# dog-qiuqiu/Yolo-FastestV2

Measured on AMD Instinct MI355X. Metric: images/sec at 352x352 bs=256 per GPU (forward+decode+NMS), higher is better.
Workload: dtype f32 tensors; contractions fp16x3 (two-term fp16 split operands on v_mfma_f32_16x16x32_f16, fp32 accumulate); depthwise/BN/ReLU/decode/NMS fp32 VALU; 1 GPU

## Files before the change

### yolo_fastestv2_amd/csrc/yfv2_block.hip

```cpp
#include <cstdlib>
#include <type_traits>

#include "yfv2_device.h"

template <int C2>
struct S1Cfg {
  static constexpr int KC = (C2 + 15) / 16;
  static constexpr int DW_FL = 9 * KC * 16;
  static constexpr int CST_FL = 6 * KC * 16;
};

constexpr int CH_TBL_FL = 64;

constexpr int CH6_WP_FL = 3 * 3 * 256;
constexpr int CH6_IMG_FL = 2 * CH6_WP_FL + S1Cfg<48>::DW_FL + S1Cfg<48>::CST_FL + CH_TBL_FL;

__host__ __device__ constexpr int s1chain_pitch(int PW) { return 2 * (PW + 1) + ((PW - 2 * (PW + 1)) % 16 + 16) % 16; }
__host__ __device__ constexpr int s1chain_plane(int PH, int PW) { return (2 * (PH + 1) * s1chain_pitch(PW) + 15) & ~15; }

template <int THREADS>
__global__ __launch_bounds__(THREADS, 2) void block_s1chain6_kernel(BlockS1Args a) {
  constexpr int C2 = 48;
  using Cfg = S1Cfg<C2>;
  constexpr int KC = Cfg::KC, NQ = C2 / 4, C = 2 * C2, NT = 4;
// ... 66 lines not shown
#undef CH6_EACH
  };

  auto phase_a = [&]() __attribute__((always_inline)) {
    BOps b[NT];
    int slo[NT];
#pragma unroll
    for (int n = 0; n < NT; ++n) slo[n] = opq(sl[n]);
#pragma unroll
    for (int n = 0; n < NT; ++n) {
      f32x4 bf[KC];
#pragma unroll
      for (int s2 = 0; s2 < KC; ++s2) bf[s2] = *reinterpret_cast<const f32x4*>(Tg + ((size_t)(4 * s2) * PL + slo[n]) * 4);
      b[n] = make_b(bf[0], bf[1], bf[2]);
    }
#pragma unroll
    for (int mt = 0; mt < KC; ++mt) {
      f32x4 acc[NT];
#pragma unroll
      for (int n = 0; n < NT; ++n) acc[n] = (f32x4){0.f, 0.f, 0.f, 0.f};
      mfma9(W1P, mt, b, acc);
      if (mt == 0) { watch.see(acc[0][0]); watch.see(acc[1][0]); watch.see(acc[2][0]); watch.see(acc[3][0]); }
      const f32x4 sc1 = *reinterpret_cast<const f32x4*>(CS + 0 * KC * 16 + 16 * mt + 4 * g);
      const f32x4 sh1 = *reinterpret_cast<const f32x4*>(CS + 1 * KC * 16 + 16 * mt + 4 * g);
      if (pvalid) {
#pragma unroll
        for (int n = 0; n < NT; ++n) {
          f32x4 y;
#pragma unroll
          for (int c = 0; c < 4; ++c) {
            const float uu = __builtin_fmaf(acc[n][c], sc1[c], sh1[c]);
            y[c] = uu > 0.f ? uu : 0.f;
          }
          *reinterpret_cast<f32x4*>(T1 + ((size_t)(4 * mt + g) * PL + slo[n]) * 4) = y;
        }
      }
      __builtin_amdgcn_sched_barrier(0);
    }
  };
  const int wro[4] = {0, (PH + 1) * RPT, RPT, (PH + 2) * RPT};
  const int wco[4] = {0, CP1, 1, CP1 + 1};
  auto phase_b = [&](f32x4 (&bo)[KC][NT]) __attribute__((always_inline)) {
    f32x4 dwv[KC][NT];
    const int wb = opq(wbase);
#pragma unroll
    for (int s = 0; s < KC; ++s) {
      const int cb = 16 * s + 4 * g;
      f32x4 wl[9];
#pragma unroll
      for (int k = 0; k < 9; ++k) wl[k] = *reinterpret_cast<const f32x4*>(WD + k * KC * 16 + cb);
      const f32x4 lsc = *reinterpret_cast<const f32x4*>(CS + 2 * KC * 16 + cb);
      const f32x4 lsh = *reinterpret_cast<const f32x4*>(CS + 3 * KC * 16 + cb);
      const float* pl = Tg + ((size_t)(4 * s) * PL + wb) * 4;
      f32x4 d[NT];
#pragma unroll
      for (int n = 0; n < NT; ++n) d[n] = (f32x4){0.f, 0.f, 0.f, 0.f};
#pragma unroll
      for (int wr = 0; wr < 4; ++wr) {
        f32x4 row[4];
#pragma unroll
        for (int wc = 0; wc < 4; ++wc) row[wc] = *reinterpret_cast<const f32x4*>(pl + (size_t)(wro[wr] + wco[wc]) * 4);
#pragma unroll
        for (int dy = 0; dy < 2; ++dy) {
          const int ky = wr - dy;
          if (ky < 0 || ky > 2) continue;
#pragma unroll
          for (int dx = 0; dx < 2; ++dx)
#pragma unroll
            for (int kx = 0; kx < 3; ++kx)
              d[2 * dy + dx] = __builtin_elementwise_fma(row[dx + kx], wl[3 * ky + kx], d[2 * dy + dx]);
        }
      }
#pragma unroll
      for (int n = 0; n < NT; ++n) dwv[s][n] = __builtin_elementwise_fma(d[n], lsc, lsh);
      __builtin_amdgcn_sched_barrier(0);
    }
    BOps b[NT];
#pragma unroll
    for (int n = 0; n < NT; ++n) b[n] = make_b(dwv[0][n], dwv[1][n], dwv[2][n]);
#pragma unroll
    for (int mt = 0; mt < KC; ++mt) {
      f32x4 acc[NT];
#pragma unroll
      for (int n = 0; n < NT; ++n) acc[n] = (f32x4){0.f, 0.f, 0.f, 0.f};
      mfma9(W2P, mt, b, acc);
      if (mt == 0) { watch.see(acc[0][0]); watch.see(acc[1][0]); watch.see(acc[2][0]); watch.see(acc[3][0]); }
      const f32x4 sc = *reinterpret_cast<const f32x4*>(CS + 4 * KC * 16 + 16 * mt + 4 * g);
      const f32x4 sh = *reinterpret_cast<const f32x4*>(CS + 5 * KC * 16 + 16 * mt + 4 * g);
#pragma unroll
      for (int n = 0; n < NT; ++n)
#pragma unroll
        for (int k = 0; k < 4; ++k) {
          const float u = __builtin_fmaf(acc[n][k], sc[k], sh[k]);
          bo[mt][n][k] = u > 0.f ? u : 0.f;
        }
      __builtin_amdgcn_sched_barrier(0);
    }
  };
  auto write_tile = [&](int nt, f32x4 q0, f32x4 q1, f32x4 q2) __attribute__((always_inline)) {
    if (!real[nt]) { q0 = (f32x4){0.f, 0.f, 0.f, 0.f}; q1 = q0; q2 = q0; }
    const int so = opq(sl[nt]);
    *reinterpret_cast<f32x4*>(T1 + ((size_t)(0 + g) * PL + so) * 4) = q0;
    *reinterpret_cast<f32x4*>(T1 + ((size_t)(4 + g) * PL + so) * 4) = q1;
    *reinterpret_cast<f32x4*>(T1 + ((size_t)(8 + g) * PL + so) * 4) = q2;
  };
  auto tbl = [&](int i) __attribute__((always_inline)) {
    return reinterpret_cast<const int*>(IM + 2 * CH6_WP_FL + Cfg::DW_FL + Cfg::CST_FL)[i * 4 + g];
  };
  constexpr int P1_4 = CH6_WP_FL / 4, P2_4 = (CH6_IMG_FL - CH6_WP_FL) / 4;
  constexpr int NI1 = (P1_4 + THREADS - 1) / THREADS, NI2 = (P2_4 + THREADS - 1) / THREADS;
  auto part_issue = [&](int kb_next, int off4, int n4, auto& regs) __attribute__((always_inline)) {
    const f32x4* src = reinterpret_cast<const f32x4*>(a.img + (size_t)(kb_next < NB ? kb_next : 0) * CH6_IMG_FL) + off4;
#pragma unroll
    for (int k = 0; k < (int)(sizeof(regs) / sizeof(regs[0])); ++k) { const int i = tid + k * THREADS; regs[k] = src[i < n4 ? i : n4 - 1]; }
  };
  auto part_commit = [&](int off4, int n4, const auto& regs) __attribute__((always_inline)) {
    __builtin_amdgcn_s_waitcnt(0x0F70);
#pragma unroll
    for (int k = 0; k < (int)(sizeof(regs) / sizeof(regs[0])); ++k) { const int i = tid + k * THREADS; if (i < n4) reinterpret_cast<f32x4*>(IM)[off4 + i] = regs[k]; }
  };

  for (int b = blockIdx.x; b < a.B; b += gridDim.x) {
    const float* ximg = a.in + (size_t)b * HW * C;
    float* zimg = a.out + (size_t)b * HW * C;
    float* pimg = a.park + (size_t)b * NPARK * PP4;
    float hold2[6][NT];
    {
      f32x4 xq[NT][6];
#pragma unroll
      for (int nt = 0; nt < NT; ++nt)
#pragma unroll
        for (int c = 0; c < 6; ++c)
          xq[nt][c] = *reinterpret_cast<const f32x4*>(ximg + (size_t)pix[nt] * C + 16 * c + 4 * g);
      {
        f32x4 i1[NI1], i2[NI2];
        part_issue(0, 0, P1_4, i1);
        part_issue(0, P1_4, P2_4, i2);
        __builtin_amdgcn_sched_barrier(0);
        part_commit(0, P1_4, i1);
        part_commit(P1_4, P2_4, i2);
      }
#pragma unroll
      for (int nt = 0; nt < NT; ++nt) {
        if (!real[nt]) {
#pragma unroll
          for (int c = 0; c < 6; ++c) xq[nt][c] = (f32x4){0.f, 0.f, 0.f, 0.f};
        }
        if (valid[nt]) {
#pragma unroll
          for (int j = 0; j < KC; ++j)
            *reinterpret_cast<f32x4*>(T1 + ((size_t)(4 * j + g) * PL + sl[nt]) * 4) = (f32x4){xq[nt][2 * j][1], xq[nt][2 * j][3], xq[nt][2 * j + 1][1], xq[nt][2 * j + 1][3]};
        }
#pragma unroll
        for (int c = 0; c < 6; ++c) hold2[c][nt] = xq[nt][c][2];
      }
      YFV2_WSTAMP(12);
      lds_barrier();
      YFV2_WSTAMP(13);
#pragma unroll
      for (int c = 0; c < 6; ++c) {
        const int pos = tbl(3 + c);
        if (pvalid) {
          if (pos < NPARK) {
            *reinterpret_cast<f32x4*>(pimg + (size_t)pos * PP4 + 4 * patch) = (f32x4){xq[0][c][0], xq[1][c][0], xq[2][c][0], xq[3][c][0]};
          } else {
#pragma unroll
            for (int nt = 0; nt < NT; ++nt) zimg[(size_t)pix[nt] * C + pos] = xq[nt][c][0];
          }
        }
      }
    }
    YFV2_WSTAMP(1);

    f32x4 bo[KC][NT];
    float Hd[KC][NT];
    auto run_block = [&](const int kb, auto first_tag) __attribute__((always_inline)) {
      constexpr bool FIRST = decltype(first_tag)::value;
      const bool more = kb + 1 < NB;
      {
        f32x4 n1[NI1];
        part_issue(kb + 1, 0, P1_4, n1);
        __builtin_amdgcn_sched_barrier(0);
        phase_a();
        __builtin_amdgcn_sched_barrier(0);
        if (kb == 1) YFV2_WSTAMP(6);
        if (FIRST) YFV2_WSTAMP(2);
        lds_barrier();
        if (kb == 1) YFV2_WSTAMP(7);
        if (FIRST) YFV2_WSTAMP(3);
        __builtin_amdgcn_s_waitcnt(0x0F70);
        if (more) part_commit(0, P1_4, n1);
      }
      const int ps0 = tbl(0), ps1 = tbl(1), ps2 = tbl(2);
      f32x4 n2[NI2];
      part_issue(kb + 1, P1_4, P2_4, n2);
      float plq[3][NT];
      if constexpr (!FIRST) {
        if (more) {
#pragma unroll
          for (int i = 0; i < 3; ++i) {
            const float* rec = pimg + (size_t)(12 * (kb - 1) + 3 * g + i) * PP4;
#pragma unroll
            for (int nt = 0; nt < NT; ++nt) plq[i][nt] = rec[opq(4 * patch + nt)];
          }
        }
      }
      __builtin_amdgcn_sched_barrier(0);
      phase_b(bo);
      if (kb == 1) YFV2_WSTAMP(8);
      if (FIRST) YFV2_WSTAMP(4);
      __builtin_amdgcn_s_waitcnt(0x0F70);
      if (more) {
        lds_barrier();
        part_commit(P1_4, P2_4, n2);
#pragma unroll
        for (int nt = 0; nt < NT; ++nt) {
          if (valid[nt]) {
            if constexpr (FIRST)
              write_tile(nt, (f32x4){hold2[0][nt], hold2[1][nt], hold2[2][nt], hold2[3][nt]},
                         (f32x4){hold2[4][nt], hold2[5][nt], bo[0][nt][1], bo[0][nt][3]},
                         (f32x4){bo[1][nt][1], bo[1][nt][3], bo[2][nt][1], bo[2][nt][3]});
            else
              write_tile(nt, (f32x4){Hd[0][nt], Hd[1][nt], Hd[2][nt], plq[0][nt]},
                         (f32x4){plq[1][nt], plq[2][nt], bo[0][nt][1], bo[0][nt][3]},
                         (f32x4){bo[1][nt][1], bo[1][nt][3], bo[2][nt][1], bo[2][nt][3]});
          }
#pragma unroll
          for (int mt = 0; mt < KC; ++mt) Hd[mt][nt] = bo[mt][nt][0];
        }
        if (pvalid) {
          const int ps[3] = {ps0, ps1, ps2};
#pragma unroll
          for (int i = 0; i < 3; ++i) {
            if (ps[i] < NPARK) {
              *reinterpret_cast<f32x4*>(pimg + (size_t)ps[i] * PP4 + 4 * patch) = (f32x4){bo[i][0][2], bo[i][1][2], bo[i][2][2], bo[i][3][2]};
            } else {
#pragma unroll
              for (int nt = 0; nt < NT; ++nt) zimg[(size_t)pix[nt] * C + ps[i]] = bo[i][nt][2];
            }
          }
        }
        lds_barrier();
        if (kb == 1) YFV2_WSTAMP(9);
        if (FIRST) YFV2_WSTAMP(5);
      }
    };
    run_block(0, std::true_type{});
#pragma unroll 1
    for (int kb = 1; kb < NB; ++kb) run_block(kb, std::false_type{});
    YFV2_WSTAMP(10);
#pragma unroll
    for (int nt = 0; nt < NT; ++nt)
      if (real[nt]) {
        float* zp = zimg + (size_t)pix[nt] * C;
#pragma unroll
        for (int mt = 0; mt < KC; ++mt) *reinterpret_cast<f32x4*>(zp + 16 * mt + 4 * g) = bo[mt][nt];
#pragma unroll
        for (int mt = 0; mt < KC; ++mt) zp[C2 + 3 * g + mt] = Hd[mt][nt];
      }
    YFV2_WSTAMP(11);
    __syncthreads();
  }
  watch.report(a.nonfinite);
}

static long s1chain_lds_floats(int H, int W) {
  const long pl = s1chain_plane(H / 2, W / 2);
  return (long)CH6_IMG_FL + 12L * pl * 4;
}

long yfv2_s1chain_park_floats(int H, int W, int nblk) { return 12L * (nblk - 2) * ((((H / 2) * (W / 2) + 15) & ~15) * 4); }

int yfv2_s1chain_image_floats() { return CH6_IMG_FL; }

bool yfv2_s1chain_supported(int c2, int H, int W) {
  if (c2 != 48 || H < 2 || (H & 1) || (W & 1)) return false;
  if ((H / 2) * (W / 2) > 16 * 8) return false;
  if (yfv2_s1chain_park_floats(H, W, 7) > 24L * (4 * H) * (4 * W)) return false;
  return s1chain_lds_floats(H, W) * 4 <= YFV2_LDS_FULL;
}

bool yfv2_launch_block_s1chain(const BlockS1Args& a, hipStream_t s) {
  if (!yfv2_s1chain_supported(48, a.H, a.W) || a.nblk < 2) return false;
  const size_t lds = sizeof(float) * (size_t)s1chain_lds_floats(a.H, a.W);
  const Yfv2Device dev = yfv2_device();
  YFV2_LAUNCH_LDS(dev, (block_s1chain6_kernel<512>), YFV2_LDS_FULL, dim3(yfv2_image_grid(a.B, dev)), dim3(512), lds, s, a);
  return true;
}

constexpr int P96_C2 = 96, P96_C = 192, P96_KC = 6, P96_TH = 3, P96_TC = 32;
constexpr int P96_CPP = P96_C + 4;
constexpr int P96_TP = P96_TC + 4;
constexpr int P96_W1_FL = 2 * P96_KC * 256, P96_W2_FL = P96_KC * 2 * 256;
constexpr int P96_IMG_FL = P96_W1_FL + P96_W2_FL + 9 * P96_TC + 4 * P96_TC + 2 * P96_C2;
constexpr int P96_W1P_FL = 2 * (P96_KC / 2) * 2 * 256, P96_W2P_FL = P96_KC * 1 * 2 * 256;
constexpr int P96_IMGP_FL = P96_W1P_FL + P96_W2P_FL + 9 * P96_TC + 4 * P96_TC + 2 * P96_C2;
constexpr int P96_MAXPX = 128;

template <int THREADS, bool PRE>
__global__ __launch_bounds__(THREADS, 2) void block_s1pool_kernel(BlockS1Args a) {
  constexpr int NW = THREADS / 64;
  constexpr int IMG_FL = PRE ? P96_IMGP_FL : P96_IMG_FL;
  constexpr int W1_FL = PRE ? P96_W1P_FL : P96_W1_FL, W2_FL = PRE ? P96_W2P_FL : P96_W2_FL;
  constexpr int N4 = IMG_FL / 4, NIT = (N4 + THREADS - 1) / THREADS;
  extern __shared__ __attribute__((aligned(16))) float lds[];
  float* POOL = lds;
  float* T = POOL + a.H * a.W * P96_CPP;
  float* IMG = T + (a.H + 2) * (a.W + 2) * P96_TP;
  Yfv2Watch watch;
  const int H = a.H, W = a.W, HW = H * W, WP = W + 2, NB = a.nblk;
  const float invW = 1.0f / (float)W;
  const int tid = threadIdx.x, lane = tid & 63, p = lane & 15, g = lane >> 4, wave = tid >> 6;
  const int px = 16 * wave + p;
  const bool pv = px < HW;
  const int pxc = pv ? px : HW - 1;
  const int py = yfv2_fdiv(pxc, invW), pxx = pxc - py * W;
  float* tpix = T + ((py + 1) * WP + pxx + 1) * P96_TP;
  const float* twin = T + (py * WP + pxx) * P96_TP;
  float* ppix = POOL + pxc * P96_CPP;
  static_assert(NW * 16 >= P96_MAXPX, "one tile per wave");

  YFV2_WSTAMP(0);
  for (int i = tid; i < (H + 2) * WP * P96_TP / 4; i += THREADS) reinterpret_cast<f32x4*>(T)[i] = (f32x4){0.f, 0.f, 0.f, 0.f};

  for (int b = blockIdx.x; b < a.B; b += gridDim.x) {
    {
      const f32x4* src = reinterpret_cast<const f32x4*>(a.in + (size_t)b * HW * P96_C);
      const f32x4* isrc = reinterpret_cast<const f32x4*>(a.img);
      constexpr int NPX = (P96_MAXPX * (P96_C / 4) + THREADS - 1) / THREADS;
      const int n4 = HW * (P96_C / 4);
      f32x4 ti[NIT];
#pragma unroll
      for (int k = 0; k < NIT; ++k) { const int i = tid + k * THREADS; ti[k] = i < N4 ? isrc[i] : (f32x4){0.f, 0.f, 0.f, 0.f}; }
#pragma unroll
      for (int k0 = 0; k0 < NPX; k0 += 6) {
        f32x4 tp[6];
#pragma unroll
        for (int k = 0; k < 6; ++k) { const int i = tid + (k0 + k) * THREADS; tp[k] = i < n4 ? src[i] : (f32x4){0.f, 0.f, 0.f, 0.f}; }
#pragma unroll
        for (int k = 0; k < 6; ++k) {
          const int i = tid + (k0 + k) * THREADS;
          const int ipx = i / (P96_C / 4), q = i - ipx * (P96_C / 4);
          if (i < n4) *reinterpret_cast<f32x4*>(POOL + ipx * P96_CPP + 4 * q) = tp[k];
        }
      }
#pragma unroll
      for (int k = 0; k < NIT; ++k) { const int i = tid + k * THREADS; if (i < N4) reinterpret_cast<f32x4*>(IMG)[i] = ti[k]; }
    }
    __syncthreads();
    YFV2_WSTAMP(1);

#pragma unroll 1
    for (int blk = 0; blk < NB; ++blk) {
      f32x4 acc2[P96_KC];
#pragma unroll
      for (int mt = 0; mt < P96_KC; ++mt) acc2[mt] = (f32x4){0.f, 0.f, 0.f, 0.f};
      yfv2_h8 b1a[PRE ? P96_KC / 2 : 1], b1b[PRE ? P96_KC / 2 : 1];
      auto split_pair = [&](f32x4 c0, f32x4 c1, yfv2_h8& t1, yfv2_h8& t2) __attribute__((always_inline)) {
        u32x4 u1, u2;
        const f32x4 cs[2] = {c0 * 16.0f, c1 * 16.0f};
#pragma unroll
        for (int e = 0; e < 2; ++e) {
          const u32x4 t = split_f16x2(cs[e]);
          u1[2 * e] = t[0]; u1[2 * e + 1] = t[1]; u2[2 * e] = t[2]; u2[2 * e + 1] = t[3];
        }
        t1 = __builtin_bit_cast(yfv2_h8, u1); t2 = __builtin_bit_cast(yfv2_h8, u2);
      };
      if constexpr (PRE) {
#pragma unroll
        for (int sp = 0; sp < P96_KC / 2; ++sp) {
          f32x4 c[2];
#pragma unroll
          for (int e = 0; e < 2; ++e) {
            const int s2 = 2 * sp + e;
            const f32x4 q0 = *reinterpret_cast<const f32x4*>(ppix + 32 * s2 + 8 * g);
            const f32x4 q1 = *reinterpret_cast<const f32x4*>(ppix + 32 * s2 + 8 * g + 4);
            c[e] = (f32x4){q0[1], q0[3], q1[1], q1[3]};
          }
          split_pair(c[0], c[1], b1a[sp], b1b[sp]);
        }
      }
#pragma unroll 1
      for (int th = 0; th < P96_TH; ++th) {
        const int t = blk * P96_TH + th;
        const bool more = t + 1 < NB * P96_TH;
        const float* W1t = IMG;
        const float* W2t = IMG + W1_FL;
        const float* TAPS = W2t + W2_FL;
        const float* CSV = TAPS + 9 * P96_TC;
        f32x4 nimg[NIT];
        {
          const f32x4* isrc = reinterpret_cast<const f32x4*>(a.img + (size_t)(t + 1) * IMG_FL);
#pragma unroll
          for (int k = 0; k < NIT; ++k) { const int i = tid + k * THREADS; nimg[k] = (more && i < N4) ? isrc[i] : (f32x4){0.f, 0.f, 0.f, 0.f}; }
        }
        {
          f32x4 acc1[2] = {{0.f, 0.f, 0.f, 0.f}, {0.f, 0.f, 0.f, 0.f}};
          if constexpr (PRE) {
#pragma unroll
            for (int sp = 0; sp < P96_KC / 2; ++sp) {
              yfv2_h8 a1[2], a2[2];
#pragma unroll
              for (int mt = 0; mt < 2; ++mt) {
                const float* wq2 = W1t + (((mt * (P96_KC / 2) + sp) * 2) * 64 + lane) * 4;
                a1[mt] = __builtin_bit_cast(yfv2_h8, *reinterpret_cast<const u32x4*>(wq2));
                a2[mt] = __builtin_bit_cast(yfv2_h8, *reinterpret_cast<const u32x4*>(wq2 + 256));
              }
#define P96_PROD(A_, B_) _Pragma("unroll") for (int mt = 0; mt < 2; ++mt) acc1[mt] = __builtin_amdgcn_mfma_f32_16x16x32_f16(A_[mt], B_, acc1[mt], 0, 0, 0);
              P96_PROD(a1, b1b[sp]) P96_PROD(a2, b1a[sp]) P96_PROD(a1, b1a[sp])
#undef P96_PROD
            }
            watch.see(acc1[0][0]);
          } else {
#pragma unroll
          for (int s2 = 0; s2 < P96_KC; ++s2) {
            const f32x4 q0 = *reinterpret_cast<const f32x4*>(ppix + 32 * s2 + 8 * g);
            const f32x4 q1 = *reinterpret_cast<const f32x4*>(ppix + 32 * s2 + 8 * g + 4);
            const f32x4 bf = {q0[1], q0[3], q1[1], q1[3]};
            const f32x4 a0 = *reinterpret_cast<const f32x4*>(W1t + ((0 * P96_KC + s2) * 64 + lane) * 4);
            const f32x4 a1 = *reinterpret_cast<const f32x4*>(W1t + ((1 * P96_KC + s2) * 64 + lane) * 4);
#pragma unroll
            for (int j = 0; j < 4; ++j) {
              acc1[0] = __builtin_amdgcn_mfma_f32_16x16x4f32(a0[j], bf[j], acc1[0], 0, 0, 0);
              acc1[1] = __builtin_amdgcn_mfma_f32_16x16x4f32(a1[j], bf[j], acc1[1], 0, 0, 0);
            }
          }
          }
          if (pv) {
#pragma unroll
            for (int mt = 0; mt < 2; ++mt) {
              const f32x4 sc = *reinterpret_cast<const f32x4*>(CSV + 0 * P96_TC + 16 * mt + 4 * g);
              const f32x4 sh = *reinterpret_cast<const f32x4*>(CSV + 1 * P96_TC + 16 * mt + 4 * g);
              f32x4 y;
#pragma unroll
              for (int c = 0; c < 4; ++c) { const float u = __builtin_fmaf(acc1[mt][c], sc[c], sh[c]); y[c] = u > 0.f ? u : 0.f; }
              *reinterpret_cast<f32x4*>(tpix + 16 * mt + 4 * g) = y;
            }
          }
        }
        if (blk == 0) YFV2_WSTAMP(2 + 4 * th);
        __syncthreads();
        if (blk == 0) YFV2_WSTAMP(3 + 4 * th);
        if constexpr (PRE) {
          f32x4 bfr2[2];
#pragma unroll
          for (int c2 = 0; c2 < 2; ++c2) {
            const int cb = 16 * c2 + 4 * g;
            f32x4 win[9], wl[9];
#pragma unroll
            for (int k = 0; k < 9; ++k) {
              win[k] = *reinterpret_cast<const f32x4*>(twin + ((k / 3) * WP + (k % 3)) * P96_TP + cb);
              wl[k] = *reinterpret_cast<const f32x4*>(TAPS + k * P96_TC + cb);
            }
            const f32x4 dsc = *reinterpret_cast<const f32x4*>(CSV + 2 * P96_TC + cb);
            const f32x4 dsh = *reinterpret_cast<const f32x4*>(CSV + 3 * P96_TC + cb);
            f32x4 d = {0.f, 0.f, 0.f, 0.f};
#pragma unroll
            for (int k = 0; k < 9; ++k)
#pragma unroll
              for (int c = 0; c < 4; ++c) d[c] = __builtin_fmaf(win[k][c], wl[k][c], d[c]);
#pragma unroll
            for (int c = 0; c < 4; ++c) bfr2[c2][c] = __builtin_fmaf(d[c], dsc[c], dsh[c]);
          }
          yfv2_h8 x1, x2;
          split_pair(bfr2[0], bfr2[1], x1, x2);
          yfv2_h8 a1[P96_KC], a2[P96_KC];
#pragma unroll
          for (int mt = 0; mt < P96_KC; ++mt) {
            const float* wq2 = W2t + ((mt * 2) * 64 + lane) * 4;
            a1[mt] = __builtin_bit_cast(yfv2_h8, *reinterpret_cast<const u32x4*>(wq2));
            a2[mt] = __builtin_bit_cast(yfv2_h8, *reinterpret_cast<const u32x4*>(wq2 + 256));
          }
#define P96_PROD(A_, B_) _Pragma("unroll") for (int mt = 0; mt < P96_KC; ++mt) acc2[mt] = __builtin_amdgcn_mfma_f32_16x16x32_f16(A_[mt], B_, acc2[mt], 0, 0, 0);
          P96_PROD(a1, x2) P96_PROD(a2, x1) P96_PROD(a1, x1)
#undef P96_PROD
        } else {
#pragma unroll
        for (int c2 = 0; c2 < 2; ++c2) {
          const int cb = 16 * c2 + 4 * g;
          f32x4 win[9], wl[9], af[P96_KC];
#pragma unroll
          for (int k = 0; k < 9; ++k) {
            win[k] = *reinterpret_cast<const f32x4*>(twin + ((k / 3) * WP + (k % 3)) * P96_TP + cb);
            wl[k] = *reinterpret_cast<const f32x4*>(TAPS + k * P96_TC + cb);
          }
          const f32x4 dsc = *reinterpret_cast<const f32x4*>(CSV + 2 * P96_TC + cb);
          const f32x4 dsh = *reinterpret_cast<const f32x4*>(CSV + 3 * P96_TC + cb);
#pragma unroll
          for (int mt = 0; mt < P96_KC; ++mt) af[mt] = *reinterpret_cast<const f32x4*>(W2t + ((mt * 2 + c2) * 64 + lane) * 4);
          __builtin_amdgcn_sched_barrier(0);
          f32x4 d = {0.f, 0.f, 0.f, 0.f}, bfr;
#pragma unroll
          for (int k = 0; k < 9; ++k)
#pragma unroll
            for (int c = 0; c < 4; ++c) d[c] = __builtin_fmaf(win[k][c], wl[k][c], d[c]);
#pragma unroll
          for (int c = 0; c < 4; ++c) bfr[c] = __builtin_fmaf(d[c], dsc[c], dsh[c]);
#pragma unroll
          for (int j = 0; j < 4; ++j)
#pragma unroll
            for (int mt = 0; mt < P96_KC; ++mt) acc2[mt] = __builtin_amdgcn_mfma_f32_16x16x4f32(af[mt][j], bfr[j], acc2[mt], 0, 0, 0);
        }
        }
        if (th == P96_TH - 1) {
          if constexpr (PRE) watch.see(acc2[0][0]);
#pragma unroll
          for (int mt = 0; mt < P96_KC; ++mt) {
            const f32x4 sc = *reinterpret_cast<const f32x4*>(CSV + 4 * P96_TC + 16 * mt + 4 * g);
            const f32x4 sh = *reinterpret_cast<const f32x4*>(CSV + 4 * P96_TC + P96_C2 + 16 * mt + 4 * g);
#pragma unroll
            for (int c = 0; c < 4; ++c) { const float u = __builtin_fmaf(acc2[mt][c], sc[c], sh[c]); acc2[mt][c] = u > 0.f ? u : 0.f; }
          }
        }
        if (blk == 0) YFV2_WSTAMP(4 + 4 * th);
        __syncthreads();
        if (more) {
#pragma unroll
          for (int k = 0; k < NIT; ++k) { const int i = tid + k * THREADS; if (i < N4) reinterpret_cast<f32x4*>(IMG)[i] = nimg[k]; }
        }
        if (th < P96_TH - 1) __syncthreads();
        if (blk == 0) YFV2_WSTAMP(5 + 4 * th);
      }
      {
        constexpr int NQ = P96_C2 / 4;
        constexpr int NEV = (P96_MAXPX * NQ + THREADS - 1) / THREADS;
        f32x4 ev[NEV];
#pragma unroll
        for (int k = 0; k < NEV; ++k) {
          const int i = tid + k * THREADS;
          const int ipx = i / NQ, q = i - ipx * NQ;
          ev[k] = (f32x4){0.f, 0.f, 0.f, 0.f};
          if (ipx < HW) {
            const f32x4 q0 = *reinterpret_cast<const f32x4*>(POOL + ipx * P96_CPP + 8 * q);
            const f32x4 q1 = *reinterpret_cast<const f32x4*>(POOL + ipx * P96_CPP + 8 * q + 4);
            ev[k] = (f32x4){q0[0], q0[2], q1[0], q1[2]};
          }
        }
        __syncthreads();
#pragma unroll
        for (int k = 0; k < NEV; ++k) {
          const int i = tid + k * THREADS;
          const int ipx = i / NQ, q = i - ipx * NQ;
          if (ipx < HW) *reinterpret_cast<f32x4*>(POOL + ipx * P96_CPP + 4 * q) = ev[k];
        }
        if (pv) {
#pragma unroll
          for (int mt = 0; mt < P96_KC; ++mt) *reinterpret_cast<f32x4*>(ppix + P96_C2 + 16 * mt + 4 * g) = acc2[mt];
        }
        __syncthreads();
        YFV2_WSTAMP(14 + blk);
      }
    }
    {
      f32x4* dst = reinterpret_cast<f32x4*>(a.out + (size_t)b * HW * P96_C);
      for (int i = tid; i < HW * (P96_C / 4); i += THREADS) {
        const int ipx = i / (P96_C / 4), q = i - ipx * (P96_C / 4);
        dst[i] = *reinterpret_cast<const f32x4*>(POOL + ipx * P96_CPP + 4 * q);
      }
    }
    YFV2_WSTAMP(17);
    __syncthreads();
  }
  watch.report(a.nonfinite);
}

static long s1pool_lds_floats(int H, int W, bool pre) { return (long)H * W * P96_CPP + (long)(H + 2) * (W + 2) * P96_TP + (pre ? P96_IMGP_FL : P96_IMG_FL); }
int yfv2_s1pool_image_floats(bool presplit) { return presplit ? P96_IMGP_FL : P96_IMG_FL; }
bool yfv2_s1pool_supported(int c2, int H, int W) {
  if (c2 != P96_C2 || H * W > P96_MAXPX || H * W < 1) return false;
  return s1pool_lds_floats(H, W, true) * 4 <= YFV2_LDS_FULL;
}

bool yfv2_launch_block_s1pool(const BlockS1Args& a, hipStream_t s) {
  if (!yfv2_s1pool_supported(P96_C2, a.H, a.W) || a.nblk < 1) return false;
  const size_t lds = sizeof(float) * (size_t)s1pool_lds_floats(a.H, a.W, a.presplit != 0);
  const Yfv2Device dev = yfv2_device();
  const int blocks = yfv2_image_grid(a.B, dev);
  if (a.presplit) YFV2_LAUNCH_LDS(dev, (block_s1pool_kernel<512, true>), YFV2_LDS_FULL, dim3(blocks), dim3(512), lds, s, a);
  else YFV2_LAUNCH_LDS(dev, (block_s1pool_kernel<512, false>), YFV2_LDS_FULL, dim3(blocks), dim3(512), lds, s, a);
  return true;
}

constexpr int TW_C = 72, TW_KC = 5;
constexpr int TW_WP_FL = TW_KC * TW_KC * 256;
constexpr int TW_WH_FL = TW_KC * 256;

template <int CIN>
struct S2Cfg {
  static constexpr int KC = (CIN + 15) / 16;
  static constexpr int CP = CIN + 4;
  static constexpr int W_FL = KC * KC * 256;
  static constexpr int DW_FL = 9 * KC * 16;
  static constexpr int NCS = 10;
  static constexpr int MAXP = 14;
  static constexpr int MAXT = CIN <= 24 ? 10 : 6;
};

template <int CIN, int THREADS, bool PPIN>
__global__ __launch_bounds__(THREADS) void block_s2_kernel(BlockS2Args a) {
  using Cfg = S2Cfg<CIN>;
  constexpr int KC = Cfg::KC, CP = Cfg::CP, KS = KC * 16;
  constexpr int NW = THREADS / 64;
  constexpr int CO = 2 * CIN;
  extern __shared__ __attribute__((aligned(16))) float lds[];
  float* W1 = lds;
  float* W2 = W1 + Cfg::W_FL;
  float* WJ = W2 + Cfg::W_FL;
  float* WD = WJ + Cfg::W_FL;
  float* WE = WD + Cfg::DW_FL;
  float* CS = WE + Cfg::DW_FL;
  float* T1 = CS + Cfg::NCS * KS;
  const int H = a.H, W = a.W, R = a.R, OH = H >> 1, OW = W >> 1;
  const float invW = 1.0f / (float)W, invOW = 1.0f / (float)OW;
  const int WP = W + 1;
  const int t1_fl = (2 * R + 1) * WP * CP + 16;
  const int tid = threadIdx.x, lane = tid & 63, p = lane & 15, g = lane >> 4, wave = tid >> 6;

  const int tiles_per_img = (OH + R - 1) / R;
  const int n_items = a.B * tiles_per_img;
  constexpr int QPP = CIN / 4;
  constexpr int MAXP = Cfg::MAXP;
  constexpr int NPL = CIN / 2;
  constexpr int NST = PPIN ? 2 * NPL : 2 * MAXP;
  f32x2 st[NST];
  auto stage_issue = [&](int item_, bool active) {
    const int item = active ? item_ : 0;
    const int b = item / tiles_per_img, ti = item - b * tiles_per_img;
    const int y0 = ti * R, rows = min(R, OH - y0);
    if constexpr (PPIN) {
      const int npx = active ? (2 * rows + 1) * W : 0;
      const int g0 = (2 * y0 - 1) * W;
      const bool okA = tid < npx && g0 + tid >= 0, okB = tid + THREADS < npx && g0 + tid + THREADS >= 0;
      const float* pA = a.in + (size_t)b * (size_t)a.pp_imgstride + (okA ? (size_t)(g0 + tid) * 2 : 0);
      const float* pB = a.in + (size_t)b * (size_t)a.pp_imgstride + (okB ? (size_t)(g0 + tid + THREADS) * 2 : 0);
#pragma unroll
      for (int pl = 0; pl < NPL; ++pl) {
        const size_t po = (size_t)pl * H * W * 2 + (((a.pp_mask >> pl) & 1u) ? (size_t)a.pp_bufstride : 0);
        st[2 * pl] = okA ? *reinterpret_cast<const f32x2*>(pA + po) : (f32x2){0.f, 0.f};
        st[2 * pl + 1] = okB ? *reinterpret_cast<const f32x2*>(pB + po) : (f32x2){0.f, 0.f};
      }
    } else {
      const int nq = active ? (2 * rows + 1) * W * QPP : 0;
      const size_t in_px = (size_t)b * H * W;
#pragma unroll
      for (int j = 0; j < MAXP; ++j) {
        const int i = tid + j * THREADS;
        const int pix = i / QPP, q = i - pix * QPP;
        const int r = yfv2_fdiv(pix, invW), x = pix - r * W;
        const int gy = 2 * y0 - 1 + r;
        f32x4 v = {0.f, 0.f, 0.f, 0.f};
        if (i < nq && gy >= 0 && gy < H) v = *reinterpret_cast<const f32x4*>(a.in + (in_px + (size_t)gy * W + x) * CIN + 4 * q);
        st[2 * j] = (f32x2){v[0], v[1]};
        st[2 * j + 1] = (f32x2){v[2], v[3]};
      }
    }
  };
  auto stage_commit = [&](int item) {
    const int b = item / tiles_per_img, ti = item - b * tiles_per_img;
    const int y0 = ti * R, rows = min(R, OH - y0);
    if constexpr (PPIN) {
      const int npx = (2 * rows + 1) * W;
      const int rA = yfv2_fdiv(tid, invW), xA = tid - rA * W, rB = yfv2_fdiv(tid + THREADS, invW), xB = tid + THREADS - rB * W;
      float* tA = T1 + (rA * WP + xA + 1) * CP;
      float* tB = T1 + (rB * WP + xB + 1) * CP;
      const bool okA = tid < npx, okB = tid + THREADS < npx;
#pragma unroll
      for (int pl = 0; pl < NPL; ++pl) {
        if (okA) *reinterpret_cast<f32x2*>(tA + 2 * pl) = st[2 * pl];
        if (okB) *reinterpret_cast<f32x2*>(tB + 2 * pl) = st[2 * pl + 1];
      }
    } else {
      const int nq = (2 * rows + 1) * W * QPP;
#pragma unroll
      for (int j = 0; j < MAXP; ++j) {
        const int i = tid + j * THREADS;
        if (i >= nq) continue;
        const int pix = i / QPP, q = i - pix * QPP;
        const int r = yfv2_fdiv(pix, invW), x = pix - r * W;
        *reinterpret_cast<f32x4*>(T1 + (r * WP + x + 1) * CP + 4 * q) = (f32x4){st[2 * j][0], st[2 * j][1], st[2 * j + 1][0], st[2 * j + 1][1]};
      }
    }
  };
  stage_issue(blockIdx.x, (int)blockIdx.x < n_items);

  {
    const f32x4* src = reinterpret_cast<const f32x4*>(a.img);
    f32x4* dst = reinterpret_cast<f32x4*>(lds);
    constexpr int N4 = (3 * Cfg::W_FL + 2 * Cfg::DW_FL + Cfg::NCS * KS) / 4;
    constexpr int NIT = (N4 + THREADS - 1) / THREADS;
    f32x4 tmp[NIT];
#pragma unroll
    for (int k = 0; k < NIT; ++k) { const int i = tid + k * THREADS; tmp[k] = i < N4 ? src[i] : (f32x4){0.f, 0.f, 0.f, 0.f}; }
#pragma unroll
    for (int k = 0; k < NIT; ++k) { const int i = tid + k * THREADS; if (i < N4) dst[i] = tmp[k]; }
  }
  for (int i = tid; i < t1_fl / 4; i += THREADS) reinterpret_cast<f32x4*>(T1)[i] = (f32x4){0.f, 0.f, 0.f, 0.f};
  __syncthreads();

  int it = 0;
#define S2_STAMP(k) do { if (it < 3) YFV2_WSTAMP(1 + 7 * it + (k)); } while (0)
  YFV2_WSTAMP(0);
  for (int item = blockIdx.x; item < n_items; item += gridDim.x) {
    const int b = item / tiles_per_img, ti = item - b * tiles_per_img;
    const int y0 = ti * R;
    const int rows = min(R, OH - y0);
    const int iy0 = 2 * y0 - 1;
    const size_t in_px = (size_t)b * H * W;
    const size_t out_px = (size_t)b * OH * OW;
    const int npxA = (2 * rows + 1) * W;
    const int npxB = rows * OW;

    stage_commit(item);
    __syncthreads();
    S2_STAMP(0);

    auto dw_pw_branch = [&](const int branch) {
      const float* taps = branch == 0 ? WD : WE;
      const float* wmat = branch == 0 ? W2 : WJ;
      const float* dsc_p = CS + (branch == 0 ? 2 : 6) * KS;
      const float* dsh_p = CS + (branch == 0 ? 3 : 7) * KS;
      const float* psc_p = CS + (branch == 0 ? 4 : 8) * KS;
      const float* psh_p = CS + (branch == 0 ? 5 : 9) * KS;
      for (int t = wave; t * 16 < npxB; t += NW) {
        const int q = 16 * t + p;
        const bool pv = q < npxB;
        const int qc = pv ? q : npxB - 1;
        const int r = yfv2_fdiv(qc, invOW), x = qc - r * OW;
        const int oy = y0 + r;
        const float* tp = T1 + ((2 * r) * WP + 2 * x) * CP;
        f32x4 bfr[KC];
#pragma unroll 1
        for (int s = 0; s < KC; ++s) {
          const int cb = 16 * s + 4 * g;
          f32x4 win[9], wk[9];
#pragma unroll
          for (int k = 0; k < 9; ++k) {
            win[k] = *reinterpret_cast<const f32x4*>(tp + ((k / 3) * WP + (k % 3)) * CP + cb);
            wk[k] = *reinterpret_cast<const f32x4*>(taps + k * KS + cb);
          }
          const f32x4 dsc = *reinterpret_cast<const f32x4*>(dsc_p + cb);
          const f32x4 dsh = *reinterpret_cast<const f32x4*>(dsh_p + cb);
          __builtin_amdgcn_sched_barrier(0);
          f32x4 d = {0.f, 0.f, 0.f, 0.f};
#pragma unroll
          for (int k = 0; k < 9; ++k)
#pragma unroll
            for (int c = 0; c < 4; ++c) d[c] = __builtin_fmaf(win[k][c], wk[k][c], d[c]);
          f32x4 y;
#pragma unroll
          for (int c = 0; c < 4; ++c) y[c] = cb < CIN ? __builtin_fmaf(d[c], dsc[c], dsh[c]) : 0.f;
          if (s == 0) bfr[0] = y;
          if (KC > 1 && s == 1) bfr[KC > 1 ? 1 : 0] = y;
          if (KC > 2 && s == 2) bfr[KC > 2 ? 2 : 0] = y;
        }
        float* dst = a.out + (out_px + (size_t)oy * OW + x) * CO + (branch == 0 ? CIN : 0);
        f32x4 afB[KC][KC], accB[KC];
#pragma unroll
        for (int mt = 0; mt < KC; ++mt) {
          accB[mt] = (f32x4){0.f, 0.f, 0.f, 0.f};
#pragma unroll
          for (int s = 0; s < KC; ++s) afB[mt][s] = *reinterpret_cast<const f32x4*>(wmat + ((mt * KC + s) * 64 + lane) * 4);
        }
        __builtin_amdgcn_sched_barrier(0);
#pragma unroll
        for (int s = 0; s < KC; ++s)
#pragma unroll
          for (int j = 0; j < 4; ++j)
#pragma unroll
            for (int mt = 0; mt < KC; ++mt)
              accB[mt] = __builtin_amdgcn_mfma_f32_16x16x4f32(afB[mt][s][j], bfr[s][j], accB[mt], 0, 0, 0);
#pragma unroll
        for (int mt = 0; mt < KC; ++mt) {
          const int cb = 16 * mt + 4 * g;
          if (pv && cb < CIN) {
            const f32x4 sc = *reinterpret_cast<const f32x4*>(psc_p + cb);
            const f32x4 sh = *reinterpret_cast<const f32x4*>(psh_p + cb);
            f32x4 y;
#pragma unroll
            for (int k = 0; k < 4; ++k) {
              const float u = __builtin_fmaf(accB[mt][k], sc[k], sh[k]);
              y[k] = u > 0.f ? u : 0.f;
            }
            *reinterpret_cast<f32x4*>(dst + cb) = y;
          }
        }
      }
    };

    dw_pw_branch(1);
    S2_STAMP(1);
    __syncthreads();
    S2_STAMP(2);

    {
      f32x4 aw[KC][KC], sc1[KC], sh1[KC];
#pragma unroll
      for (int mt = 0; mt < KC; ++mt) {
#pragma unroll
        for (int s = 0; s < KC; ++s) {
          const f32x4 fr = *reinterpret_cast<const f32x4*>(W1 + ((mt * KC + s) * 64 + lane) * 4);
          aw[mt][s] = fr;
        }
        sc1[mt] = *reinterpret_cast<const f32x4*>(CS + 0 * KS + 16 * mt + 4 * g);
        sh1[mt] = *reinterpret_cast<const f32x4*>(CS + 1 * KS + 16 * mt + 4 * g);
      }
      auto tile_off = [&](int t) {
        const int q = 16 * t + p;
        const int qc = q < npxA ? q : npxA - 1;
        const int r = yfv2_fdiv(qc, invW), x = qc - r * W;
        return (r * WP + x + 1) * CP;
      };
      f32x4 bf[KC], bn[KC];
      int t = wave;
      if (t * 16 < npxA) {
        const int o = tile_off(t);
#pragma unroll
        for (int s = 0; s < KC; ++s) bf[s] = (16 * s + 4 * g < CIN) ? *reinterpret_cast<const f32x4*>(T1 + o + 16 * s + 4 * g) : (f32x4){0.f, 0.f, 0.f, 0.f};
      }
      for (; t * 16 < npxA; t += NW) {
        const int tn = t + NW;
        const int on = tile_off(tn * 16 < npxA ? tn : t);
#pragma unroll
        for (int s = 0; s < KC; ++s) bn[s] = (16 * s + 4 * g < CIN) ? *reinterpret_cast<const f32x4*>(T1 + on + 16 * s + 4 * g) : (f32x4){0.f, 0.f, 0.f, 0.f};
// ... 683 lines not shown
```

### yolo_fastestv2_amd/csrc/yfv2_device.h

```cpp
#pragma once
#include "yfv2_internal.h"

typedef float f32x4 __attribute__((ext_vector_type(4)));
typedef float f32x2 __attribute__((ext_vector_type(2)));
typedef float f32x3u __attribute__((ext_vector_type(3), aligned(4)));
typedef unsigned int u32x2 __attribute__((ext_vector_type(2)));
typedef unsigned int u32x3 __attribute__((ext_vector_type(3)));
typedef unsigned int u32x4 __attribute__((ext_vector_type(4)));
typedef _Float16 yfv2_h2 __attribute__((ext_vector_type(2)));
typedef _Float16 yfv2_h4 __attribute__((ext_vector_type(4)));
typedef _Float16 yfv2_h8 __attribute__((ext_vector_type(8)));
typedef __bf16 yfv2_bf16x8 __attribute__((ext_vector_type(8)));

__device__ __forceinline__ int yfv2_fdiv(int n, float inv_d) { return (int)(((float)n + 0.5f) * inv_d); }

__device__ __forceinline__ int f2i(float v) { return __builtin_bit_cast(int, v); }
__device__ __forceinline__ float i2f(int v) { return __builtin_bit_cast(float, v); }
__device__ __forceinline__ float row_shr1(float v) {
  return __builtin_bit_cast(float, __builtin_amdgcn_update_dpp(0, __builtin_bit_cast(int, v), 0x111, 0xf, 0xf, true));
}
__device__ __forceinline__ unsigned row_shr1(unsigned v) { return (unsigned)__builtin_amdgcn_update_dpp(0, (int)v, 0x111, 0xf, 0xf, true); }
__device__ __forceinline__ float row_shl1(float v) {
  return __builtin_bit_cast(float, __builtin_amdgcn_update_dpp(0, __builtin_bit_cast(int, v), 0x101, 0xf, 0xf, true));
}
template <int K>
__device__ __forceinline__ float quad_mul(float tap4, float v) {
  return __builtin_bit_cast(float, __builtin_amdgcn_update_dpp(0, __builtin_bit_cast(int, tap4), K * 0x55, 0xf, 0xf, false)) * v;
}
#define YFV2_QP(n) "quad_perm:[%" #n ",%" #n ",%" #n ",%" #n "] row_mask:0xf bank_mask:0xf\n\t"
template <int KA>
__device__ __forceinline__ void quad_fmac1(float& s, float ta, float v) {
  asm("s_nop 1\n\tv_fmac_f32_dpp %0, %1, %2 " YFV2_QP(3) : "+v"(s) : "v"(ta), "v"(v), "n"(KA));
}
template <int KA, int KB, int KC>
__device__ __forceinline__ void quad_mul2_fmac1(float& s, float& q, float ta, float tb, float tc, float v0, float v1) {
  asm("s_nop 1\n\tv_mul_f32_dpp %0, %2, %5 " YFV2_QP(7) "v_mul_f32_dpp %1, %3, %6 " YFV2_QP(8) "v_fmac_f32_dpp %0, %4, %6 " YFV2_QP(9)
      : "=&v"(s), "=&v"(q) : "v"(ta), "v"(tb), "v"(tc), "v"(v0), "v"(v1), "n"(KA), "n"(KB), "n"(KC));
}
template <int KA, int KB, int KC>
__device__ __forceinline__ void quad_fmac3(float& s, float& q, float ta, float tb, float tc, float v0, float v1) {
  asm("s_nop 1\n\tv_fmac_f32_dpp %0, %2, %5 " YFV2_QP(7) "v_fmac_f32_dpp %1, %3, %6 " YFV2_QP(8) "v_fmac_f32_dpp %0, %4, %6 " YFV2_QP(9)
      : "+v"(s), "+v"(q) : "v"(ta), "v"(tb), "v"(tc), "v"(v0), "v"(v1), "n"(KA), "n"(KB), "n"(KC));
}
template <int K3, int K4, int K5, int K6, int K7, int K8>
__device__ __forceinline__ void quad_fmac6(float& a0, float& a1, float& a2, float t3, float t4, float t5, float t6, float t7, float t8,
                                           float u, float w) {
  asm("s_nop 1\n\tv_fmac_f32_dpp %0, %3, %9 " YFV2_QP(11) "v_fmac_f32_dpp %1, %4, %9 " YFV2_QP(12) "v_fmac_f32_dpp %2, %5, %9 " YFV2_QP(13)
      "v_fmac_f32_dpp %0, %6, %10 " YFV2_QP(14) "v_fmac_f32_dpp %1, %7, %10 " YFV2_QP(15) "v_fmac_f32_dpp %2, %8, %10 " YFV2_QP(16)
      : "+v"(a0), "+v"(a1), "+v"(a2)
      : "v"(t3), "v"(t4), "v"(t5), "v"(t6), "v"(t7), "v"(t8), "v"(u), "v"(w), "n"(K3), "n"(K4), "n"(K5), "n"(K6), "n"(K7), "n"(K8));
}
#undef YFV2_QP
__device__ __forceinline__ void dpp_src_ready(float& v) { asm volatile("s_nop 1" : "+v"(v)); }

__device__ __forceinline__ unsigned pack_hi_hi(unsigned a, unsigned b) { return __builtin_amdgcn_perm(b, a, 0x07060302u); }
__device__ __forceinline__ unsigned pack_hi_lo(unsigned a, unsigned b) { return __builtin_amdgcn_perm(b, a, 0x05040302u); }
__device__ __forceinline__ unsigned u8pair(unsigned hi, unsigned lo, unsigned sel) {
  const unsigned v = __builtin_amdgcn_perm(hi, lo, sel) | 0x64006400u;
  const yfv2_h2 h = __builtin_bit_cast(yfv2_h2, v) - (yfv2_h2){(_Float16)1024.0f, (_Float16)1024.0f};
  return __builtin_bit_cast(unsigned, h);
}

__device__ __forceinline__ u32x2 split_f16x2(f32x2 v) {
  const yfv2_h2 t1 = __builtin_convertvector(v, yfv2_h2);
  const f32x2 r = v - __builtin_convertvector(t1, f32x2);
  const yfv2_h2 t2 = __builtin_convertvector(r, yfv2_h2);
  return (u32x2){__builtin_bit_cast(unsigned, t1), __builtin_bit_cast(unsigned, t2)};
}
__device__ __forceinline__ u32x4 split_f16x2(f32x4 v) {
  const yfv2_h4 t1 = __builtin_convertvector(v, yfv2_h4);
  const f32x4 r = v - __builtin_convertvector(t1, f32x4);
  const yfv2_h4 t2 = __builtin_convertvector(r, yfv2_h4);
  const u32x2 a = __builtin_bit_cast(u32x2, t1), b = __builtin_bit_cast(u32x2, t2);
  return (u32x4){a[0], a[1], b[0], b[1]};
}

struct Row16 { unsigned p01[2], p23[2], m[2]; };
struct Row8 { unsigned p01, p23, m; };
__device__ __forceinline__ void split_cols(const f32x4 v, Row16& o) {
  const u32x2 a = split_f16x2((f32x2){v[0], v[1]} * 256.0f), b = split_f16x2((f32x2){v[2], v[3]} * 256.0f);
  o.p01[0] = a[0]; o.p01[1] = a[1];
  o.p23[0] = b[0]; o.p23[1] = b[1];
}
__device__ __forceinline__ void split_cols_u8(const u32x3 d, unsigned sel_a, unsigned sel_b, Row8& o) {
  o.p01 = u8pair(d[1], d[0], sel_a);
  o.p23 = u8pair(d[2], d[1], sel_b);
}

struct Bf3A { u32x4 hh, mm, hl; };
struct Bf3B { u32x4 hm, lh; };
__device__ __forceinline__ unsigned yfv2_pack_hi16(float a, float b) {
  return __builtin_amdgcn_perm(__builtin_bit_cast(unsigned, b), __builtin_bit_cast(unsigned, a), 0x07060302u);
}
__device__ __forceinline__ float yfv2_trunc_bf16(float a) { return __builtin_bit_cast(float, __builtin_bit_cast(unsigned, a) & 0xffff0000u); }
__device__ __forceinline__ void yfv2_split3(f32x4 v, unsigned (&h)[2], unsigned (&m)[2], unsigned (&l)[2]) {
  float r1[4], r2[4];
#pragma unroll
  for (int c = 0; c < 4; ++c) { r1[c] = v[c] - yfv2_trunc_bf16(v[c]); r2[c] = r1[c] - yfv2_trunc_bf16(r1[c]); }
  h[0] = yfv2_pack_hi16(v[0], v[1]); h[1] = yfv2_pack_hi16(v[2], v[3]);
  m[0] = yfv2_pack_hi16(r1[0], r1[1]); m[1] = yfv2_pack_hi16(r1[2], r1[3]);
  l[0] = yfv2_pack_hi16(r2[0], r2[1]); l[1] = yfv2_pack_hi16(r2[2], r2[3]);
}
__device__ __forceinline__ Bf3A yfv2_split_a(f32x4 w) {
  unsigned h[2], m[2], l[2];
  yfv2_split3(w, h, m, l);
  return {(u32x4){h[0], h[1], h[0], h[1]}, (u32x4){m[0], m[1], m[0], m[1]}, (u32x4){h[0], h[1], l[0], l[1]}};
}
__device__ __forceinline__ Bf3B yfv2_split_b(f32x4 x) {
  unsigned h[2], m[2], l[2];
  yfv2_split3(x, h, m, l);
  return {(u32x4){h[0], h[1], m[0], m[1]}, (u32x4){l[0], l[1], h[0], h[1]}};
}
template <int k>
__device__ __forceinline__ f32x4 yfv2_mfma6_step(const Bf3A& a, const Bf3B& b, f32x4 acc) {
  if constexpr (k == 0) return __builtin_amdgcn_mfma_f32_16x16x32_bf16(__builtin_bit_cast(yfv2_bf16x8, a.hl), __builtin_bit_cast(yfv2_bf16x8, b.lh), acc, 0, 0, 0);
  else if constexpr (k == 1) return __builtin_amdgcn_mfma_f32_16x16x32_bf16(__builtin_bit_cast(yfv2_bf16x8, a.mm), __builtin_bit_cast(yfv2_bf16x8, b.hm), acc, 0, 0, 0);
  else return __builtin_amdgcn_mfma_f32_16x16x32_bf16(__builtin_bit_cast(yfv2_bf16x8, a.hh), __builtin_bit_cast(yfv2_bf16x8, b.hm), acc, 0, 0, 0);
}
template <int MT_, int NT_>
__device__ __forceinline__ void yfv2_mfma6_tiles(const Bf3A (&a)[MT_], const Bf3B (&b)[NT_], f32x4 (&acc)[MT_][NT_]) {
#pragma unroll
  for (int mt = 0; mt < MT_; ++mt)
#pragma unroll
    for (int nt = 0; nt < NT_; ++nt) acc[mt][nt] = yfv2_mfma6_step<0>(a[mt], b[nt], acc[mt][nt]);
#pragma unroll
  for (int mt = 0; mt < MT_; ++mt)
#pragma unroll
    for (int nt = 0; nt < NT_; ++nt) acc[mt][nt] = yfv2_mfma6_step<1>(a[mt], b[nt], acc[mt][nt]);
#pragma unroll
  for (int mt = 0; mt < MT_; ++mt)
#pragma unroll
    for (int nt = 0; nt < NT_; ++nt) acc[mt][nt] = yfv2_mfma6_step<2>(a[mt], b[nt], acc[mt][nt]);
}

struct Yfv2Watch {
  unsigned long long m = 0;
  __device__ __forceinline__ void see(float v) {
    const unsigned b = __builtin_bit_cast(unsigned, v);
    m |= __builtin_amdgcn_ballot_w64((b << 1) >= 0xff000000u);
  }
  __device__ __forceinline__ void report(int* flag) const {
    if (m != 0 && flag != nullptr) *reinterpret_cast<volatile int*>(flag) = 1;
  }
};

__device__ __forceinline__ float sigmoid_f32(float x) { return __fdiv_rn(1.0f, __fadd_rn(1.0f, expf(-x))); }
template <int MAXPER>
__device__ __forceinline__ void yfv2_softmax_quad(const float* cls, int nc, int hw, int cc, int part, float (&ev)[MAXPER]) {
  const int per = (nc + 3) >> 2;
  const int c_lo = part * per, c_hi = min(nc, c_lo + per);
  float lv[MAXPER];
#pragma unroll
  for (int i = 0; i < MAXPER; ++i) {
    const int c = c_lo + i;
    lv[i] = cls[(unsigned)((c < c_hi ? c : (c_lo < nc ? c_lo : 0)) * hw + cc)];
  }
  float m = -INFINITY;
#pragma unroll
  for (int i = 0; i < MAXPER; ++i)
    if (c_lo + i < c_hi) m = fmaxf(m, lv[i]);
  m = fmaxf(m, __shfl_xor(m, 1));
  m = fmaxf(m, __shfl_xor(m, 2));
  float sum = 0.f;
#pragma unroll
  for (int i = 0; i < MAXPER; ++i) {
    ev[i] = 0.f;
    if (c_lo + i < c_hi) {
      ev[i] = expf(__fsub_rn(lv[i], m));
      sum = __fadd_rn(sum, ev[i]);
    }
  }
  sum = __fadd_rn(sum, __shfl_xor(sum, 1));
  sum = __fadd_rn(sum, __shfl_xor(sum, 2));
#pragma unroll
  for (int i = 0; i < MAXPER; ++i) ev[i] = __fdiv_rn(ev[i], sum);
}

template <typename T>
__device__ __forceinline__ T wave_fold(T v) {
#pragma unroll
  for (int off = 32; off >= 1; off >>= 1) v += __shfl_xor(v, off, 64);
  return v;
}

#define YFV2_STAMP(i) do { if (a.trace && blockIdx.x == 0 && threadIdx.x == 0) a.trace[i] = (long long)__builtin_readcyclecounter(); } while (0)
#define YFV2_WSTAMP(i) do { if (a.trace && blockIdx.x == 0 && (threadIdx.x & 63) == 0) a.trace[64 + 32 * (threadIdx.x >> 6) + (i)] = (long long)__builtin_readcyclecounter(); } while (0)
```

Before: 468,200 images/s.

## Stage per-tile weights into LDS via direct global_load_lds in split phases

Replaces the register-staged prefetch of the next tile's weight image (global load into VGPRs, then LDS store) with direct global-to-LDS loads. The next image is now copied in two parts: W1 and the first scale/shift rows after the first-conv barrier, and the rest after the second barrier. This drops one barrier per tile. It removes the register pressure and the VALU/LDS store traffic of the prefetch, which may help occupancy. In exchange the load latency is no longer hidden behind compute, because of the explicit vmcnt waits before the barriers, and the split-region ordering must exactly match which parts each phase still reads.

```diff
diff --git a/yolo_fastestv2_amd/csrc/yfv2_block.hip b/yolo_fastestv2_amd/csrc/yfv2_block.hip
--- a/yolo_fastestv2_amd/csrc/yfv2_block.hip
+++ b/yolo_fastestv2_amd/csrc/yfv2_block.hip
@@ -392,7 +392,9 @@
   constexpr int NW = THREADS / 64;
   constexpr int IMG_FL = PRE ? P96_IMGP_FL : P96_IMG_FL;
   constexpr int W1_FL = PRE ? P96_W1P_FL : P96_W1_FL, W2_FL = PRE ? P96_W2P_FL : P96_W2_FL;
-  constexpr int N4 = IMG_FL / 4, NIT = (N4 + THREADS - 1) / THREADS;
+  constexpr int N4 = IMG_FL / 4;
+  constexpr int CS_OFF = W1_FL + W2_FL + 9 * P96_TC;
+  static_assert(IMG_FL % 4 == 0 && W1_FL % 4 == 0 && CS_OFF % 4 == 0 && P96_TC % 2 == 0, "16-byte runs");
   extern __shared__ __attribute__((aligned(16))) float lds[];
   float* POOL = lds;
   float* T = POOL + a.H * a.W * P96_CPP;
@@ -416,12 +418,9 @@
   for (int b = blockIdx.x; b < a.B; b += gridDim.x) {
     {
       const f32x4* src = reinterpret_cast<const f32x4*>(a.in + (size_t)b * HW * P96_C);
-      const f32x4* isrc = reinterpret_cast<const f32x4*>(a.img);
+      yfv2_lds_stage<THREADS>(IMG, a.img, N4);
       constexpr int NPX = (P96_MAXPX * (P96_C / 4) + THREADS - 1) / THREADS;
       const int n4 = HW * (P96_C / 4);
-      f32x4 ti[NIT];
-#pragma unroll
-      for (int k = 0; k < NIT; ++k) { const int i = tid + k * THREADS; ti[k] = i < N4 ? isrc[i] : (f32x4){0.f, 0.f, 0.f, 0.f}; }
 #pragma unroll
       for (int k0 = 0; k0 < NPX; k0 += 6) {
         f32x4 tp[6];
@@ -434,9 +433,8 @@
           if (i < n4) *reinterpret_cast<f32x4*>(POOL + ipx * P96_CPP + 4 * q) = tp[k];
         }
       }
-#pragma unroll
-      for (int k = 0; k < NIT; ++k) { const int i = tid + k * THREADS; if (i < N4) reinterpret_cast<f32x4*>(IMG)[i] = ti[k]; }
-    }
+    }
+    __builtin_amdgcn_s_waitcnt(0x0F70);
     __syncthreads();
     YFV2_WSTAMP(1);
 
@@ -478,12 +476,7 @@
         const float* W2t = IMG + W1_FL;
         const float* TAPS = W2t + W2_FL;
         const float* CSV = TAPS + 9 * P96_TC;
-        f32x4 nimg[NIT];
-        {
-          const f32x4* isrc = reinterpret_cast<const f32x4*>(a.img + (size_t)(t + 1) * IMG_FL);
-#pragma unroll
-          for (int k = 0; k < NIT; ++k) { const int i = tid + k * THREADS; nimg[k] = (more && i < N4) ? isrc[i] : (f32x4){0.f, 0.f, 0.f, 0.f}; }
-        }
+        const float* nsrc = a.img + (size_t)(t + 1) * IMG_FL;
         {
           f32x4 acc1[2] = {{0.f, 0.f, 0.f, 0.f}, {0.f, 0.f, 0.f, 0.f}};
           if constexpr (PRE) {
@@ -529,7 +522,12 @@
           }
         }
         if (blk == 0) YFV2_WSTAMP(2 + 4 * th);
+        __builtin_amdgcn_s_waitcnt(0x0F70);
         __syncthreads();
+        if (more) {
+          yfv2_lds_stage<THREADS>(IMG, nsrc, W1_FL / 4);
+          yfv2_lds_stage<THREADS>(IMG + CS_OFF, nsrc + CS_OFF, 2 * P96_TC / 4);
+        }
         if (blk == 0) YFV2_WSTAMP(3 + 4 * th);
         if constexpr (PRE) {
           f32x4 bfr2[2];
@@ -603,12 +601,12 @@
           }
         }
         if (blk == 0) YFV2_WSTAMP(4 + 4 * th);
+        __builtin_amdgcn_s_waitcnt(0x0F70);
         __syncthreads();
         if (more) {
-#pragma unroll
-          for (int k = 0; k < NIT; ++k) { const int i = tid + k * THREADS; if (i < N4) reinterpret_cast<f32x4*>(IMG)[i] = nimg[k]; }
-        }
-        if (th < P96_TH - 1) __syncthreads();
+          yfv2_lds_stage<THREADS>(IMG + W1_FL, nsrc + W1_FL, (CS_OFF - W1_FL) / 4);
+          yfv2_lds_stage<THREADS>(IMG + CS_OFF + 2 * P96_TC, nsrc + CS_OFF + 2 * P96_TC, (IMG_FL - CS_OFF - 2 * P96_TC) / 4);
+        }
         if (blk == 0) YFV2_WSTAMP(5 + 4 * th);
       }
       {
diff --git a/yolo_fastestv2_amd/csrc/yfv2_device.h b/yolo_fastestv2_amd/csrc/yfv2_device.h
--- a/yolo_fastestv2_amd/csrc/yfv2_device.h
+++ b/yolo_fastestv2_amd/csrc/yfv2_device.h
@@ -183,5 +183,16 @@
   return v;
 }
 
+template <int THREADS>
+__device__ __forceinline__ void yfv2_lds_stage(float* lds_dst, const float* gsrc, int n4) {
+  const int tid = threadIdx.x;
+  const int w0 = __builtin_amdgcn_readfirstlane(tid & ~63);
+#pragma unroll
+  for (int k = 0; k < n4; k += THREADS)
+    if (k + tid < n4)
+      __builtin_amdgcn_global_load_lds((const __attribute__((address_space(1))) void*)(gsrc + 4 * (size_t)(k + tid)),
+                                       (__attribute__((address_space(3))) void*)(lds_dst + 4 * (k + w0)), 16, 0, 0);
+}
+
 #define YFV2_STAMP(i) do { if (a.trace && blockIdx.x == 0 && threadIdx.x == 0) a.trace[i] = (long long)__builtin_readcyclecounter(); } while (0)
 #define YFV2_WSTAMP(i) do { if (a.trace && blockIdx.x == 0 && (threadIdx.x & 63) == 0) a.trace[64 + 32 * (threadIdx.x >> 6) + (i)] = (long long)__builtin_readcyclecounter(); } while (0)
```

Result: no change. 468,400 images/s, median of 5 (+0.0%).
